# JasperSnoek/spearmint

Hardware: NVIDIA H100
Metric: EI candidates/sec (higher is better)
Workload: dtype f32

## Files before the change

### spearmint_b200/csrc/predict_tc.cu

```cuda
#include <cuda_fp16.h>
#include <cuda.h>

#include <algorithm>
#include <vector>
#include <cstdlib>
#include <cstring>

#include "common.cuh"
#include "tc_common.cuh"

namespace smk {

__global__ void __launch_bounds__(256, 2) trtri_finalize_kernel(int Npad, int ldx, int K, const float* __restrict__ winv,
                                                                 float* X) {
  using C = Cfg<float>;
  constexpr int NB = C::NB, TM = C::TM, TN = C::TN;
  extern __shared__ __align__(16) unsigned char smem_raw[];
  TileSmem<float>& sm = *reinterpret_cast<TileSmem<float>*>(smem_raw);
  float (*Ts)[NB + kPad] = reinterpret_cast<float (*)[NB + kPad]>(smem_raw + sizeof(TileSmem<float>));
  const int nblk = Npad / NB, J = blockIdx.x, s = blockIdx.y;
  const int tid = threadIdx.x, ty = tid >> 4, tx = tid & 15;
  const float* W = winv + ((long)s * nblk + K) * NB * NB;
  float* Xt = X + (long)s * ldx * ldx + (long)K * NB * ldx + (long)J * NB;
  float acc[TM][TN];
// ... 77 lines not shown
  long e = (long)blockIdx.x * blockDim.x + threadIdx.x;
  if (e >= total) return;
  long per = (long)ld * ld;
  int r = (int)((e % per) / ld), c = (int)(e % ld);
  float x = (c <= r && r < Npad) ? X[e] : 0.f;
  float h = tf32_hi(x);
  hi[e] = h;
  lo[e] = x - h;
}

__global__ void __launch_bounds__(256) linv_mv_kernel(int N, int Np, const float* __restrict__ hi,
                                                      const float* __restrict__ lo, const float* __restrict__ y,
                                                      const float* __restrict__ mean, float* __restrict__ t) {
  const int s = blockIdx.y, warp = threadIdx.x >> 5, lane = threadIdx.x & 31;
  const int row = blockIdx.x * 8 + warp;
  if (row >= Np) return;
  const long base = ((long)s * Np + row) * Np;
  const float mu = mean[s];
  float acc = 0.f;
  for (int k = lane; k <= row && k < N; k += 32) acc = fmaf(hi[base + k] + lo[base + k], y[k] - mu, acc);
#pragma unroll
  for (int o = 16; o > 0; o >>= 1) acc += __shfl_xor_sync(0xffffffffu, acc, o);
  if (lane == 0) t[(long)s * Np + row] = (row < N) ? acc : 0.f;
}
__global__ void __launch_bounds__(256) linv_mtv_kernel(int N, int Np, int ld_alpha, const float* __restrict__ hi,
                                                       const float* __restrict__ lo, const float* __restrict__ t,
                                                       float* __restrict__ alpha) {
  __shared__ float red[4][64];
  const int s = blockIdx.y, cl = threadIdx.x & 63, ph = threadIdx.x >> 6;
  const int c = blockIdx.x * 64 + cl;
  const float* th = t + (long)s * Np;
  const long base = (long)s * Np * Np + c;
  float acc = 0.f;
  if (c < N)
    for (int r = (c & ~3) + ph; r < N; r += 4)
      if (r >= c) acc = fmaf(hi[base + (long)r * Np] + lo[base + (long)r * Np], th[r], acc);
  red[ph][cl] = acc;
  __syncthreads();
  if (ph == 0 && c < ld_alpha) alpha[(long)s * ld_alpha + c] = (c < N) ? red[0][cl] + red[1][cl] + red[2][cl] + red[3][cl] : 0.f;
}

__global__ void __launch_bounds__(256) linv_absmax_kernel(long per4, const float4* __restrict__ hi,
                                                          const float4* __restrict__ lo, unsigned* __restrict__ maxbits) {
  const int s = blockIdx.y;
  const float4* h = hi + (long)s * per4;
  const float4* l = lo + (long)s * per4;
  float m = 0.f;
  for (long e = (long)blockIdx.x * blockDim.x + threadIdx.x; e < per4; e += (long)gridDim.x * blockDim.x) {
    float4 a = h[e], b = l[e];
    m = fmaxf(m, fmaxf(fmaxf(fabsf(a.x + b.x), fabsf(a.y + b.y)), fmaxf(fabsf(a.z + b.z), fabsf(a.w + b.w))));
  }
#pragma unroll
  for (int o = 16; o > 0; o >>= 1) m = fmaxf(m, __shfl_xor_sync(0xffffffffu, m, o));
  if ((threadIdx.x & 31) == 0) atomicMax(&maxbits[s], __float_as_uint(m));
}

__global__ void __launch_bounds__(256) linv_pack_f16_kernel(long per4, const float4* __restrict__ hi,
                                                            const float4* __restrict__ lo,
                                                            const unsigned* __restrict__ maxbits, uint2* __restrict__ oh,
                                                            uint2* __restrict__ ol, int* __restrict__ exps) {
  const int s = blockIdx.y;
  const int eb = scale_exp(__uint_as_float(maxbits[s]));
  const float sc = ldexpf(1.f, eb);
  if (blockIdx.x == 0 && threadIdx.x == 0) exps[s] = eb;
  const long base = (long)s * per4;
  for (long e = (long)blockIdx.x * blockDim.x + threadIdx.x; e < per4; e += (long)gridDim.x * blockDim.x) {
    float4 a = hi[base + e], b = lo[base + e];
    __half hh[4], ll[4];
    split16((a.x + b.x) * sc, hh[0], ll[0]);
    split16((a.y + b.y) * sc, hh[1], ll[1]);
    split16((a.z + b.z) * sc, hh[2], ll[2]);
    split16((a.w + b.w) * sc, hh[3], ll[3]);
    oh[base + e] = pack4(hh);
    ol[base + e] = pack4(ll);
  }
}

__global__ void __launch_bounds__(256) alpha_absmax_kernel(int N, int F, int Npad_alpha, const float* __restrict__ alpha,
                                                           int* __restrict__ fexp) {
  __shared__ float red[8];
  const int s = blockIdx.x;
  float m = 0.f;
  for (long e = threadIdx.x; e < (long)F * N; e += blockDim.x) {
    int f = (int)(e / N), n = (int)(e % N);
    m = fmaxf(m, fabsf(alpha[((long)s * F + f) * Npad_alpha + n]));
  }
#pragma unroll
  for (int o = 16; o > 0; o >>= 1) m = fmaxf(m, __shfl_xor_sync(0xffffffffu, m, o));
  if ((threadIdx.x & 31) == 0) red[threadIdx.x >> 5] = m;
  __syncthreads();
  if (threadIdx.x == 0) {
    for (int w = 1; w < 8; ++w) m = fmaxf(m, red[w]);
    fexp[s] = scale_exp(m);
  }
}
__global__ void alpha_pack_f16_kernel(int N, int Np, int F, int Fp, int Npad_alpha, long total,
                                      const float* __restrict__ alpha, const int* __restrict__ fexp,
                                      __half* __restrict__ hi, __half* __restrict__ lo) {
  long e = (long)blockIdx.x * blockDim.x + threadIdx.x;
  if (e >= total) return;
  int n = (int)(e % Np);
  long sf = e / Np;
  int f = (int)(sf % Fp), s = (int)(sf / Fp);
  float x = (f < F && n < N) ? alpha[((long)s * F + f) * Npad_alpha + n] * ldexpf(1.f, fexp[s]) : 0.f;
  split16(x, hi[e], lo[e]);
}

// ... 86 lines not shown
          hh[q] = __floats2half2_rn(v.x, v.y);
          const float2 hf = __half22float2(hh[q]);
          ll[q] = __floats2half2_rn(v.x - hf.x, v.y - hf.y);
        }
        uint2 ph, pl;
        ph.x = *reinterpret_cast<unsigned*>(&hh[0]); ph.y = *reinterpret_cast<unsigned*>(&hh[1]);
        pl.x = *reinterpret_cast<unsigned*>(&ll[0]); pl.y = *reinterpret_cast<unsigned*>(&ll[1]);
        *reinterpret_cast<uint2*>(khi + ok + g * 64 + tx * 4) = ph;
        *reinterpret_cast<uint2*>(klo + ok + g * 64 + tx * 4) = pl;
      }
    }
  }
  if (!al) return;
  __syncthreads();
#pragma unroll
  for (int r = 0; r < 8; ++r) red[tx][tile_row(ty, r)] = mdot[r].x + mdot[r].y;
  __syncthreads();
  if (tid < T) {
    float v = 0.f;
    for (int q = 0; q < 16; ++q) v += red[q][tid];
    int gc = c_begin + c0 + tid;
    if (gc < M) mu[(long)s * ldm + gc] = fmaf(a2, v, mean[s]);
  }
}

namespace tc {
constexpr int BM = 128;
constexpr int BN = 256;
constexpr int BK = 16;
constexpr int BK16 = 32;
constexpr int STAGES = 4;
constexpr int ROW_BYTES = BK * 4;
static_assert(ROW_BYTES == 64 && BK16 * 2 == ROW_BYTES, "operand rows must be one 64B swizzle span in both element types");
constexpr int UK_BYTES = 32;
constexpr int A_BYTES = BM * ROW_BYTES;
constexpr int B_BYTES = BN * ROW_BYTES;
constexpr int STAGE_BYTES = 2 * A_BYTES + 2 * B_BYTES;
constexpr int CONSUMERS = 2;
constexpr int THREADS = (CONSUMERS + 1) * 128;
constexpr int PRODUCER_REGS = 40, CONSUMER_REGS = 232;
static_assert(128 * PRODUCER_REGS + CONSUMERS * 128 * CONSUMER_REGS <= 65536, "register file");
constexpr int SMEM_BYTES = STAGES * STAGE_BYTES + 1024  + 256 ;

struct Args {
  int S, Np, Mc, ntiles, npairs, ngroups, ldp;
  float* partial;
  const float* z;
  float* mpartial;
  float* dbg;
  int F, M, c_begin, ldm;
  const float* mean;
  float* mu_f;
  int f16;
  int a_evict_first;
  const float* amp2;
  const int* bexp;
  int mode;
  int Npad, jb, ncols;
  float* Cmat;
  int K;
  float *xhi, *xlo, *xthi, *xtlo;
};

struct Item { int valid, own, rowA, rowB, k0, nk, s, tile, g, pr; };

template <int CLUSTER>
__device__ __forceinline__ long num_items(const Args& p) {
  return p.mode <= 1 ? (long)p.S * ((p.ntiles + CLUSTER - 1) / CLUSTER) * p.npairs : (long)p.S * p.ntiles;
}
template <int CLUSTER>
__device__ __forceinline__ Item get_item(const Args& p, long w, int h, int rank) {
  Item it;
  it.valid = 0; it.own = 1; it.rowA = it.rowB = it.k0 = it.nk = it.s = it.tile = it.g = it.pr = 0;
  const int bk = p.f16 ? BK16 : BK;
  if (p.mode <= 1) {
    const int ntg = (p.ntiles + CLUSTER - 1) / CLUSTER;
    it.pr = (int)(w % p.npairs);
    const long st = w / p.npairs;
    it.tile = (int)(st % ntg) * CLUSTER + rank;
    it.s = (int)(st / ntg);
    if (it.tile >= p.ntiles) { it.tile = p.ntiles - 1; it.own = 0; }
    it.g = (h == 0) ? it.pr : p.ngroups - 1 - it.pr;
    if (h == 1 && (p.mode == 1 || it.g == it.pr)) return it;
    it.nk = (p.mode == 1) ? p.Np / bk : (it.g + 1) * (BN / bk);
    it.rowA = it.s * p.Mc + it.tile * BM;
    it.rowB = (it.s * p.ngroups + it.g) * BN;
    it.valid = 1;
  } else if (p.mode == 2) {
    if (h == 1) return it;
    it.tile = (int)(w % p.ntiles);
    it.s = (int)(w / p.ntiles);
    it.rowA = it.s * p.Npad + (p.jb + it.tile) * BM;
    it.rowB = it.s * p.Npad + p.jb * BM;
    it.nk = p.jb * BM / bk;
    it.valid = 1;
  } else {
    if (h == 1) return it;
    it.tile = (int)(w % p.ntiles);
    it.s = (int)(w / p.ntiles);
    it.rowA = it.s * BM;
    it.rowB = it.s * p.Np + it.tile * BN;
    it.k0 = it.tile * BN;
    it.nk = (p.K * BM - it.tile * BN) / bk;
    it.valid = 1;
  }
  return it;
}

template <int CLUSTER>
__global__ void __launch_bounds__(THREADS, 1)
predict_tc_kernel(const __grid_constant__ CUtensorMap mAhi, const __grid_constant__ CUtensorMap mAlo,
                  const __grid_constant__ CUtensorMap mBhi, const __grid_constant__ CUtensorMap mBlo, Args p) {
  static_assert(CLUSTER == 1 || CLUSTER == 2, "one CTA, or a pair sharing the B operand");
  extern __shared__ unsigned char smem_raw[];
  unsigned char* base = smem_raw + ((1024u - (smem_u32(smem_raw) & 1023u)) & 1023u);
  uint64_t* bars = reinterpret_cast<uint64_t*>(base + STAGES * STAGE_BYTES);
  uint64_t* full = bars;
  uint64_t* empty = bars + STAGES;

  const int warp = threadIdx.x >> 5, lane = threadIdx.x & 31;
  const int rank = CLUSTER > 1 ? (int)cluster_ctarank() : 0;
  if (threadIdx.x == 0) {
    for (int i = 0; i < STAGES; ++i) { mbar_init(&full[i], 1); mbar_init(&empty[i], CLUSTER * CONSUMERS * 4); }
    asm volatile("fence.mbarrier_init.release.cluster;" ::: "memory");
  }
  if (CLUSTER > 1) cluster_sync();
  else __syncthreads();

  const long nitems = num_items<CLUSTER>(p);
  const long w0 = blockIdx.x / CLUSTER, dw = gridDim.x / CLUSTER;
  const int bk = p.f16 ? BK16 : BK;
  if (warp < 4) {
    asm volatile("setmaxnreg.dec.sync.aligned.u32 %0;" ::"n"(PRODUCER_REGS));
    if (warp == 0 && lane == 0) {
      const uint64_t hintA = (p.mode == 0 && !p.a_evict_first) ? 0x1000000000000000ull : 0x12F0000000000000ull;
      const uint64_t hintB = 0x14F0000000000000ull;
      int stage = 0;
      uint32_t phase = 0;
      for (long w = w0; w < nitems; w += dw) {
        for (int h = 0; h < 2; ++h) {
          const Item it = get_item<CLUSTER>(p, w, h, rank);
          if (!it.valid) break;
          for (int kc = 0; kc < it.nk; ++kc) {
            mbar_wait_relaxed(&empty[stage], phase ^ 1, 64);
            unsigned char* sb = base + stage * STAGE_BYTES;
            const int kk = it.k0 + kc * bk;
            mbar_expect_tx(&full[stage], STAGE_BYTES);
            tma_load_2d(&mAhi, &full[stage], sb, kk, it.rowA, hintA);
            tma_load_2d(&mAlo, &full[stage], sb + A_BYTES, kk, it.rowA, hintA);
            if (CLUSTER == 1) {
              tma_load_2d(&mBhi, &full[stage], sb + 2 * A_BYTES, kk, it.rowB, hintB);
              tma_load_2d(&mBlo, &full[stage], sb + 2 * A_BYTES + B_BYTES, kk, it.rowB, hintB);
            } else {
              const int hb = rank * (BN / CLUSTER);
              const uint16_t all = (1u << CLUSTER) - 1;
              tma_load_2d_multicast(&mBhi, &full[stage], sb + 2 * A_BYTES + hb * ROW_BYTES, kk, it.rowB + hb, all, hintB);
              tma_load_2d_multicast(&mBlo, &full[stage], sb + 2 * A_BYTES + B_BYTES + hb * ROW_BYTES, kk, it.rowB + hb,
                                    all, hintB);
            }
            if (++stage == STAGES) { stage = 0; phase ^= 1; }
          }
        }
      }
    }
    if (CLUSTER > 1) cluster_sync();
    return;
  }

  asm volatile("setmaxnreg.inc.sync.aligned.u32 %0;" ::"n"(CONSUMER_REGS));
  const int wg = (warp >> 2) - 1;
  const int r0 = wg * 64 + (warp & 3) * 16 + (lane >> 2);
  const int cq = 2 * (lane & 3);
  const uint32_t a_off = (uint32_t)wg * 64 * ROW_BYTES;
  auto release = [&](int st) {
    if (CLUSTER == 1) mbar_arrive(&empty[st]);
    else
#pragma unroll
      for (int r = 0; r < CLUSTER; ++r) mbar_arrive_cluster(&empty[st], r);
  };
  float d[BN / 2];
  int stage = 0;
  uint32_t phase = 0;
  for (long w = w0; w < nitems; w += dw) {
    float acc[2] = {0.f, 0.f}, accm[2] = {0.f, 0.f};
    const Item it0 = get_item<CLUSTER>(p, w, 0, rank);
    for (int h = 0; h < 2; ++h) {
      const Item it = get_item<CLUSTER>(p, w, h, rank);
      if (!it.valid) break;
      int prev = -1;
      for (int kc = 0; kc < it.nk; ++kc) {
        mbar_wait(&full[stage], phase);
        const uint32_t sa = smem_u32(base + stage * STAGE_BYTES);
        const uint64_t ahi = wgmma_desc_sw64(sa + a_off), alo = wgmma_desc_sw64(sa + A_BYTES + a_off);
        const uint64_t bhi = wgmma_desc_sw64(sa + 2 * A_BYTES), blo = wgmma_desc_sw64(sa + 2 * A_BYTES + B_BYTES);
        wgmma_fence();
        if (p.f16) {
#pragma unroll
          for (int k = 0; k < ROW_BYTES / UK_BYTES; ++k) {
            const uint64_t ko = (uint64_t)((k * UK_BYTES) >> 4);
            wgmma_f16_n256(d, alo + ko, bhi + ko, (kc | k) ? 1u : 0u);
            wgmma_f16_n256(d, ahi + ko, blo + ko, 1u);
            wgmma_f16_n256(d, ahi + ko, bhi + ko, 1u);
          }
        } else {
#pragma unroll
          for (int k = 0; k < ROW_BYTES / UK_BYTES; ++k) {
            const uint64_t ko = (uint64_t)((k * UK_BYTES) >> 4);
            wgmma_tf32_n256(d, alo + ko, bhi + ko, (kc | k) ? 1u : 0u);
            wgmma_tf32_n256(d, ahi + ko, blo + ko, 1u);
            wgmma_tf32_n256(d, ahi + ko, bhi + ko, 1u);
          }
        }
        wgmma_commit();
        wgmma_wait<1>();
        if (prev >= 0 && lane == 0) release(prev);
        prev = stage;
        if (++stage == STAGES) { stage = 0; phase ^= 1; }
      }
      wgmma_wait<0>();
      wgmma_hold(d);
      if (prev >= 0 && lane == 0) release(prev);
      if (!it.own) continue;
      const float scl = p.f16 ? ldexpf(1.f, -(kx_exp(p.amp2[it.s]) + p.bexp[it.s])) : 1.f;
      if (p.mode == 0) {
        const float* zrow = p.z ? p.z + (long)it.s * p.Np + it.g * BN : nullptr;
#pragma unroll
        for (int nb = 0; nb < BN / 8; ++nb) {
          const int c = nb * 8 + cq;
          const float2 z2 = zrow ? __ldg(reinterpret_cast<const float2*>(zrow + c)) : make_float2(0.f, 0.f);
#pragma unroll
          for (int rh = 0; rh < 2; ++rh) {
            const float v0 = d[nb * 4 + rh * 2] * scl, v1 = d[nb * 4 + rh * 2 + 1] * scl;
            acc[rh] = fmaf(v0, v0, acc[rh]);
            acc[rh] = fmaf(v1, v1, acc[rh]);
            accm[rh] = fmaf(v0, z2.x, accm[rh]);
            accm[rh] = fmaf(v1, z2.y, accm[rh]);
            if (p.dbg) {
              float* o = p.dbg + ((long)it.s * p.Mc + it.tile * BM + r0 + 8 * rh) * p.Np + it.g * BN + c;
              o[0] = v0;
              o[1] = v1;
            }
          }
        }
      } else if (p.mode == 1) {
        const float mu0 = p.mean[it.s];
#pragma unroll
        for (int rh = 0; rh < 2; ++rh) {
          const int gc = p.c_begin + it.tile * BM + r0 + 8 * rh;
          if (gc >= p.M) continue;
#pragma unroll
          for (int nb = 0; nb < BN / 8; ++nb)
#pragma unroll
            for (int e = 0; e < 2; ++e) {
              const int f = it.g * BN + nb * 8 + cq + e;
              if (f < p.F) p.mu_f[((long)it.s * p.F + f) * p.ldm + gc] = fmaf(d[nb * 4 + rh * 2 + e], scl, mu0);
            }
        }
      } else if (p.mode == 2) {
#pragma unroll
        for (int nb = 0; nb < BN / 8; ++nb) {
          const int c = nb * 8 + cq;
          if (c >= p.ncols) continue;
#pragma unroll
          for (int rh = 0; rh < 2; ++rh) {
            float2* cp = reinterpret_cast<float2*>(
// ... 238 lines not shown
  for (int r = 0; r < TM; ++r)
#pragma unroll
    for (int c = 0; c < TN; ++c) acc[r][c] = 0.f;
  TileGemm<float, Lay::KContig, Lay::MContig, false>::run(acc, W, NB, Lk, Npad, NB, sm);
  const long off = (long)s * NB * Npad + (long)J * NB;
#pragma unroll
  for (int r = 0; r < TM; ++r)
#pragma unroll
    for (int g = 0; g < TN / 4; ++g) {
      V4<float> h, l;
#pragma unroll
      for (int e = 0; e < 4; ++e) {
        float x = acc[r][g * 4 + e];
        h.v[e] = tf32_hi(x);
        l.v[e] = tf32_lo(x, h.v[e]);
      }
      const long o = off + (long)tile_row(ty, r) * Npad + g * 64 + tx * 4;
      st4(lthi + o, h);
      st4(ltlo + o, l);
    }
}

__global__ void trtri_diag_store_kernel(int Npad, int Np, int K, const float* __restrict__ winv, float* __restrict__ xhi,
                                        float* __restrict__ xlo, float* __restrict__ xthi, float* __restrict__ xtlo) {
  constexpr int NB = 128;
  const int s = blockIdx.y, nblk = Npad / NB;
  const float* W = winv + ((long)s * nblk + K) * NB * NB;
  for (int e = blockIdx.x * blockDim.x + threadIdx.x; e < NB * NB; e += gridDim.x * blockDim.x) {
    int i = e / NB, k = e % NB;
    float x = W[e], h = tf32_hi(x), l = x - h;
    long o = ((long)s * Np + (long)K * NB + i) * Np + (long)K * NB + k;
    long ot = ((long)s * Np + (long)K * NB + k) * Np + (long)K * NB + i;
    xhi[o] = h; xlo[o] = l; xthi[ot] = h; xtlo[ot] = tf32_lo(x, h);
  }
}

size_t trtri_tc_workspace_bytes(int Npad, int Np, int S) {
  return (2 * (size_t)S * Np * Np + 2 * (size_t)S * 128 * Npad) * sizeof(float);
}

int potrf_lower_batched_tc(int, int, float*, float*, int*, float*, float*, cudaStream_t, cudaEvent_t*);
void potrf_winv_block(int, int, int, const float*, float*, cudaStream_t);

static int trtri_tc_run(int Npad, int Np, int S, const float* L, float* winv, float* linv_hi, float* linv_lo,
                        void* workspace, size_t workspace_bytes, cudaStream_t st, cudaEvent_t* blk_done) {
  if (Npad <= 0 || Npad % kNpadMult) return -1;
  if (Np < Npad || Np % tc::BN) return -2;
  if (S <= 0) return -3;
  if (!L || !winv || !linv_hi || !linv_lo) return -4;
  if (!workspace || workspace_bytes < trtri_tc_workspace_bytes(Npad, Np, S)) return -8;
  float* xthi = reinterpret_cast<float*>(workspace);
  float* xtlo = xthi + (size_t)S * Np * Np;
  float* lthi = xtlo + (size_t)S * Np * Np;
  float* ltlo = lthi + (size_t)S * 128 * Npad;
  const size_t xb = (size_t)S * Np * Np * sizeof(float);
  cudaMemsetAsync(linv_hi, 0, xb, st);
  cudaMemsetAsync(linv_lo, 0, xb, st);
  cudaMemsetAsync(xthi, 0, 2 * xb, st);
  CUtensorMap mAhi, mAlo, mBhi, mBlo;
  if (tc::make_map(&mAhi, lthi, (uint64_t)S * 128, Npad, tc::BM) || tc::make_map(&mAlo, ltlo, (uint64_t)S * 128, Npad, tc::BM) ||
      tc::make_map(&mBhi, xthi, (uint64_t)S * Np, Np, tc::BN) || tc::make_map(&mBlo, xtlo, (uint64_t)S * Np, Np, tc::BN))
    return 1999;
  static bool attr = false;
  if (!attr) {
    cudaFuncSetAttribute(tc::predict_tc_kernel<1>, cudaFuncAttributeMaxDynamicSharedMemorySize, tc::SMEM_BYTES);
    attr = true;
  }
  const int nblk = Npad / 128;
  timing_begin("trtri_kernel", st);
  for (int K = 0; K < nblk; ++K) {
    if (blk_done) {
      cudaStreamWaitEvent(st, blk_done[K], 0);
      potrf_winv_block(Npad, S, K, L, winv, st);
    }
    trtri_diag_store_kernel<<<dim3(8, S), 256, 0, st>>>(Npad, Np, K, winv, linv_hi, linv_lo, xthi, xtlo);
    count_launch();
    if (K == 0) continue;
    trtri_lt_kernel<<<dim3(K, S), 256, 0, st>>>(Npad, K, L, winv, lthi, ltlo);
    tc::Args a;
    tc_args_init(a);
    a.mode = 3; a.S = S; a.Np = Np; a.Npad = Npad; a.K = K;
    a.ntiles = (K * 128 + tc::BN - 1) / tc::BN; a.npairs = 1; a.ngroups = 1;
    a.xhi = linv_hi; a.xlo = linv_lo; a.xthi = xthi; a.xtlo = xtlo;
    long nitems = (long)S * a.ntiles;
    int grid = (int)std::min<long>(nitems, num_sms());
    tc::predict_tc_kernel<1><<<grid, tc::THREADS, tc::SMEM_BYTES, st>>>(mAhi, mAlo, mBhi, mBlo, a);
    count_launch(2);
  }
  timing_end(st);
  return check_launch("trtri_split_tc");
}
// ... 7 lines not shown
                   float* linv_lo, void* tws, size_t tws_bytes, cudaStream_t st) {
  if (Npad <= 0 || Npad % kNpadMult) return -1;
  static cudaStream_t aux = nullptr;
  static cudaEvent_t ev_in = nullptr, ev_out = nullptr;
  static std::vector<cudaEvent_t> blk;
  if (!aux) {
    cudaStreamCreateWithFlags(&aux, cudaStreamNonBlocking);
    cudaEventCreateWithFlags(&ev_in, cudaEventDisableTiming);
    cudaEventCreateWithFlags(&ev_out, cudaEventDisableTiming);
  }
  const int nblk = Npad / 128;
  while ((int)blk.size() < nblk) {
    cudaEvent_t e;
    cudaEventCreateWithFlags(&e, cudaEventDisableTiming);
    blk.push_back(e);
  }
  cudaEventRecord(ev_in, st);
  cudaStreamWaitEvent(aux, ev_in, 0);
  int rc = potrf_lower_batched_tc(Npad, S, A, winv, info, lhi, llo, st, blk.data());
  if (rc) return rc;
  rc = trtri_tc_run(Npad, Np, S, A, winv, linv_hi, linv_lo, tws, tws_bytes, aux, blk.data());
  cudaEventRecord(ev_out, aux);
  cudaStreamWaitEvent(st, ev_out, 0);
  return rc;
}

int linv_pack_f16(int Np, int S, const float* linv_hi, const float* linv_lo, __half* out_hi, __half* out_lo, int* exps,
                  cudaStream_t st) {
  if (Np <= 0 || Np % tc::BN) return -1;
  if (S <= 0) return -2;
  if (!linv_hi || !linv_lo || !out_hi || !out_lo || !exps) return -3;
  unsigned* maxbits = reinterpret_cast<unsigned*>(exps + S);
  cudaMemsetAsync(maxbits, 0, sizeof(unsigned) * S, st);
  const long per4 = (long)Np * Np / 4;
  const int gx = (int)std::min<long>((per4 + 255) / 256, 4L * num_sms());
  timing_begin("linv_pack_f16", st);
  linv_absmax_kernel<<<dim3(gx, S), 256, 0, st>>>(per4, reinterpret_cast<const float4*>(linv_hi),
                                                  reinterpret_cast<const float4*>(linv_lo), maxbits);
  linv_pack_f16_kernel<<<dim3(gx, S), 256, 0, st>>>(per4, reinterpret_cast<const float4*>(linv_hi),
                                                    reinterpret_cast<const float4*>(linv_lo), maxbits,
                                                    reinterpret_cast<uint2*>(out_hi), reinterpret_cast<uint2*>(out_lo), exps);
  timing_end(st);
  count_launch(2);
  return check_launch("linv_pack_f16");
}

int linv_alpha(int N, int Np, int S, const float* linv_hi, const float* linv_lo, const float* y, const float* mean,
               float* alpha, int ld_alpha, float* tmp, cudaStream_t st) {
  if (N <= 0 || Np < N) return -1;
  if (S <= 0) return -3;
  if (!linv_hi || !linv_lo || !y || !mean || !alpha || !tmp) return -4;
  if (ld_alpha < N) return -9;
  linv_mv_kernel<<<dim3((Np + 7) / 8, S), 256, 0, st>>>(N, Np, linv_hi, linv_lo, y, mean, tmp);
  linv_mtv_kernel<<<dim3((ld_alpha + 63) / 64, S), 256, 0, st>>>(N, Np, ld_alpha, linv_hi, linv_lo, tmp, alpha);
  count_launch(2);
  return check_launch("linv_alpha");
}

static bool tc_overlap_enabled() {
  static int v = -1;
  if (v < 0) { const char* e = getenv("SMK_TC_OVERLAP"); v = (e && e[0] == '1') ? 1 : 0; }
  return v == 1;
}
static size_t tc_chunk_cands(int Np, int M, int S, size_t budget) {
  size_t per_cand = (size_t)S * Np * 2 * sizeof(__half);
  size_t mpad = ((size_t)M + 127) / 128 * 128;
  size_t mc = budget / per_cand;
  if (mc >= mpad) return mpad;
  if (tc_overlap_enabled()) mc = (budget / 2) / per_cand;
  mc = mc / 128 * 128;
  if (mc < 128) mc = 128;
  return mc;
// ... 140 lines not shown
  void* kws = reinterpret_cast<void*>(fexp + S);
  float* mu_partial = gen_tc ? kxt_tc_mu_partial(kws, Np, Mc, S, M, D) : nullptr;
  const float* gen_alpha = z ? nullptr : alpha;
  const bool pre = pregenerated && z && nbuf == 1 && g_pregen.valid && g_pregen.ws == workspace && g_pregen.M == M &&
                   g_pregen.S == S && g_pregen.Np == Np && g_pregen.N == N;
  if (pregenerated && !pre) return -21;
  if (g_pregen.valid && g_pregen.ws == workspace) {
    cudaStreamWaitEvent(st, g_pregen.done, 0);
    g_pregen.valid = false;
  }
  if (!pre && gen_tc) {
    int rc = kxt_tc_prepare(kws, N, Np, M, Mc, D, S, X, Cc, st);
    if (rc) return rc;
  }
  CUtensorMap mFhi, mFlo;
  if (fant) {
    const long total = (long)S * Fp * Np;
    alpha_absmax_kernel<<<S, 256, 0, st>>>(N, F, Npad_alpha, alpha_f, fexp);
    alpha_pack_f16_kernel<<<(unsigned)((total + 255) / 256), 256, 0, st>>>(N, Np, F, Fp, Npad_alpha, total, alpha_f, fexp,
                                                                           ahi, alo);
    count_launch(2);
    if (tc::make_map_h(&mFhi, ahi, (uint64_t)S * Fp, Np, tc::BN / tc::kPredictCluster) ||
        tc::make_map_h(&mFlo, alo, (uint64_t)S * Fp, Np, tc::BN / tc::kPredictCluster))
      return 1999;
  }

  CUtensorMap mAhi[2], mAlo[2], mBhi, mBlo;
  for (int b = 0; b < nbuf; ++b) {
    __half* kh = kbase + (size_t)b * 2 * kelems;
    if (tc::make_map_h(&mAhi[b], kh, (uint64_t)S * Mc, Np, tc::BM) ||
        tc::make_map_h(&mAlo[b], kh + kelems, (uint64_t)S * Mc, Np, tc::BM))
      return 1999;
  }
  if (tc::make_map_h(&mBhi, linv_hi, (uint64_t)S * Np, Np, tc::BN / tc::kPredictCluster) ||
      tc::make_map_h(&mBlo, linv_lo, (uint64_t)S * Np, Np, tc::BN / tc::kPredictCluster))
    return 1999;
  static cudaStream_t aux = nullptr;
  static cudaEvent_t ev_fork = nullptr, ev_kxt[2] = {nullptr, nullptr}, ev_mma[2] = {nullptr, nullptr};
  if (!aux) {
    cudaStreamCreateWithFlags(&aux, cudaStreamNonBlocking);
    cudaEventCreateWithFlags(&ev_fork, cudaEventDisableTiming);
    for (int i = 0; i < 2; ++i) {
      cudaEventCreateWithFlags(&ev_kxt[i], cudaEventDisableTiming);
      cudaEventCreateWithFlags(&ev_mma[i], cudaEventDisableTiming);
    }
  }
  const bool overlap = (nbuf == 2);
  cudaStream_t kst = overlap ? aux : st;
  if (overlap) {
    cudaEventRecord(ev_fork, st);
    cudaStreamWaitEvent(aux, ev_fork, 0);
  }
  int ci = 0;
  for (int c_begin = 0; c_begin < M; c_begin += Mc, ++ci) {
    const int b = overlap ? (ci & 1) : 0;
    __half* kh = kbase + (size_t)b * 2 * kelems;
    const int mc_used = min(Mc, ((M - c_begin) + 127) / 128 * 128);
    if (overlap && ci >= 2) cudaStreamWaitEvent(aux, ev_mma[b], 0);
    if (!(pre && ci == 0)) {
      timing_begin("kxt_kernel", kst);
      if (gen_tc) {
        int rc = kxt_tc(kws, kind, N, Np, M, c_begin, Mc, mc_used, D, S, inv_ls, amp2, gen_alpha, Npad_alpha, kh, kh + kelems, kst);
        if (rc) return rc;
      } else {
        kxt_kernel<<<dim3(mc_used / 128, S), 256, 0, kst>>>(kind, N, Np, M, c_begin, Mc, D, X, Cc, inv_ls, amp2, mean,
                                                            gen_alpha, Npad_alpha, kh, kh + kelems, mu, ldm);
      }
      timing_end(kst);
// ... 36 lines not shown
```

### spearmint_b200/csrc/tc_common.cuh

```cuda
#pragma once
#include <cuda_fp16.h>
#include <cuda.h>

#include <cstdint>

namespace smk {

__host__ __device__ __forceinline__ int scale_exp(float amax) {
  int e;
  frexpf(amax * 1.00001f, &e);
  return 15 - e;
}
__device__ __forceinline__ int kx_exp(float amp2) { return scale_exp(amp2 * 1.000001f); }
__device__ __forceinline__ void split16(float x, __half& h, __half& l) {
  h = __float2half_rn(x);
  l = __float2half_rn(x - __half2float(h));
}
__device__ __forceinline__ uint2 pack4(const __half (&v)[4]) {
  __half2 a = __halves2half2(v[0], v[1]), b = __halves2half2(v[2], v[3]);
  uint2 r;
  r.x = *reinterpret_cast<unsigned*>(&a);
  r.y = *reinterpret_cast<unsigned*>(&b);
  return r;
}
// ... 149 lines not shown
      : "l"(a), "l"(b), "r"(scale_d));
}
__device__ __forceinline__ void wgmma_tf32_n256(float (&d)[128], uint64_t a, uint64_t b, uint32_t scale_d) {
  asm volatile(
      "{\n\t.reg .pred p;\n\t"
      "setp.ne.b32 p, %130, 0;\n\t"
      "wgmma.mma_async.sync.aligned.m64n256k8.f32.tf32.tf32 "
      "{%0, %1, %2, %3, %4, %5, %6, %7, %8, %9, %10, %11, %12, %13, %14, %15, "
      "%16, %17, %18, %19, %20, %21, %22, %23, %24, %25, %26, %27, %28, %29, %30, %31, "
      "%32, %33, %34, %35, %36, %37, %38, %39, %40, %41, %42, %43, %44, %45, %46, %47, "
      "%48, %49, %50, %51, %52, %53, %54, %55, %56, %57, %58, %59, %60, %61, %62, %63, "
      "%64, %65, %66, %67, %68, %69, %70, %71, %72, %73, %74, %75, %76, %77, %78, %79, "
      "%80, %81, %82, %83, %84, %85, %86, %87, %88, %89, %90, %91, %92, %93, %94, %95, "
      "%96, %97, %98, %99, %100, %101, %102, %103, %104, %105, %106, %107, %108, %109, %110, %111, "
      "%112, %113, %114, %115, %116, %117, %118, %119, %120, %121, %122, %123, %124, %125, %126, %127}, "
      "%128, %129, p, 1, 1;\n\t}"
      : "+f"(d[0]), "+f"(d[1]), "+f"(d[2]), "+f"(d[3]), "+f"(d[4]), "+f"(d[5]), "+f"(d[6]), "+f"(d[7]), "+f"(d[8]), "+f"(d[9]), "+f"(d[10]), "+f"(d[11]), "+f"(d[12]), "+f"(d[13]), "+f"(d[14]), "+f"(d[15]), "+f"(d[16]), "+f"(d[17]), "+f"(d[18]), "+f"(d[19]), "+f"(d[20]), "+f"(d[21]), "+f"(d[22]), "+f"(d[23]), "+f"(d[24]), "+f"(d[25]), "+f"(d[26]), "+f"(d[27]), "+f"(d[28]), "+f"(d[29]), "+f"(d[30]), "+f"(d[31]), "+f"(d[32]), "+f"(d[33]), "+f"(d[34]), "+f"(d[35]), "+f"(d[36]), "+f"(d[37]), "+f"(d[38]), "+f"(d[39]), "+f"(d[40]), "+f"(d[41]), "+f"(d[42]), "+f"(d[43]), "+f"(d[44]), "+f"(d[45]), "+f"(d[46]), "+f"(d[47]), "+f"(d[48]), "+f"(d[49]), "+f"(d[50]), "+f"(d[51]), "+f"(d[52]), "+f"(d[53]), "+f"(d[54]), "+f"(d[55]), "+f"(d[56]), "+f"(d[57]), "+f"(d[58]), "+f"(d[59]), "+f"(d[60]), "+f"(d[61]), "+f"(d[62]), "+f"(d[63]), "+f"(d[64]), "+f"(d[65]), "+f"(d[66]), "+f"(d[67]), "+f"(d[68]), "+f"(d[69]), "+f"(d[70]), "+f"(d[71]), "+f"(d[72]), "+f"(d[73]), "+f"(d[74]), "+f"(d[75]), "+f"(d[76]), "+f"(d[77]), "+f"(d[78]), "+f"(d[79]), "+f"(d[80]), "+f"(d[81]), "+f"(d[82]), "+f"(d[83]), "+f"(d[84]), "+f"(d[85]), "+f"(d[86]), "+f"(d[87]), "+f"(d[88]), "+f"(d[89]), "+f"(d[90]), "+f"(d[91]), "+f"(d[92]), "+f"(d[93]), "+f"(d[94]), "+f"(d[95]), "+f"(d[96]), "+f"(d[97]), "+f"(d[98]), "+f"(d[99]), "+f"(d[100]), "+f"(d[101]), "+f"(d[102]), "+f"(d[103]), "+f"(d[104]), "+f"(d[105]), "+f"(d[106]), "+f"(d[107]), "+f"(d[108]), "+f"(d[109]), "+f"(d[110]), "+f"(d[111]), "+f"(d[112]), "+f"(d[113]), "+f"(d[114]), "+f"(d[115]), "+f"(d[116]), "+f"(d[117]), "+f"(d[118]), "+f"(d[119]), "+f"(d[120]), "+f"(d[121]), "+f"(d[122]), "+f"(d[123]), "+f"(d[124]), "+f"(d[125]), "+f"(d[126]), "+f"(d[127])
      : "l"(a), "l"(b), "r"(scale_d));
}
__device__ __forceinline__ void wgmma_f16_n128(float (&d)[64], uint64_t a, uint64_t b, uint32_t scale_d) {
  asm volatile(
      "{\n\t.reg .pred p;\n\t"
      "setp.ne.b32 p, %66, 0;\n\t"
      "wgmma.mma_async.sync.aligned.m64n128k16.f32.f16.f16 "
      "{%0, %1, %2, %3, %4, %5, %6, %7, %8, %9, %10, %11, %12, %13, %14, %15, "
      "%16, %17, %18, %19, %20, %21, %22, %23, %24, %25, %26, %27, %28, %29, %30, %31, "
      "%32, %33, %34, %35, %36, %37, %38, %39, %40, %41, %42, %43, %44, %45, %46, %47, "
      "%48, %49, %50, %51, %52, %53, %54, %55, %56, %57, %58, %59, %60, %61, %62, %63}, "
      "%64, %65, p, 1, 1, 0, 0;\n\t}"
      : "+f"(d[0]), "+f"(d[1]), "+f"(d[2]), "+f"(d[3]), "+f"(d[4]), "+f"(d[5]), "+f"(d[6]), "+f"(d[7]), "+f"(d[8]), "+f"(d[9]), "+f"(d[10]), "+f"(d[11]), "+f"(d[12]), "+f"(d[13]), "+f"(d[14]), "+f"(d[15]), "+f"(d[16]), "+f"(d[17]), "+f"(d[18]), "+f"(d[19]), "+f"(d[20]), "+f"(d[21]), "+f"(d[22]), "+f"(d[23]), "+f"(d[24]), "+f"(d[25]), "+f"(d[26]), "+f"(d[27]), "+f"(d[28]), "+f"(d[29]), "+f"(d[30]), "+f"(d[31]), "+f"(d[32]), "+f"(d[33]), "+f"(d[34]), "+f"(d[35]), "+f"(d[36]), "+f"(d[37]), "+f"(d[38]), "+f"(d[39]), "+f"(d[40]), "+f"(d[41]), "+f"(d[42]), "+f"(d[43]), "+f"(d[44]), "+f"(d[45]), "+f"(d[46]), "+f"(d[47]), "+f"(d[48]), "+f"(d[49]), "+f"(d[50]), "+f"(d[51]), "+f"(d[52]), "+f"(d[53]), "+f"(d[54]), "+f"(d[55]), "+f"(d[56]), "+f"(d[57]), "+f"(d[58]), "+f"(d[59]), "+f"(d[60]), "+f"(d[61]), "+f"(d[62]), "+f"(d[63])
      : "l"(a), "l"(b), "r"(scale_d));
}

}
}
```

### spearmint_b200/engine.py

```python
import ctypes as C
import os

import numpy as np
import scipy.stats as sps
import torch

from . import _lib
from ._lib import KINDS, check, fn, ptr

JITTER = 1e-6
CONSTRAINT_NOISE = 1e-3


def _ceil(x, m):
    return ((x + m - 1) // m) * m


class HyperBatch(object):

    def __init__(self, hyper_samples, kind, device, dtype):
        S = len(hyper_samples)
        D = len(np.atleast_1d(hyper_samples[0][3]))
        mean = np.array([h[0] for h in hyper_samples], dtype=np.float64)
        noise = np.array([h[1] for h in hyper_samples], dtype=np.float64)
# ... 4 lines not shown
        host = np.concatenate([mean, noise, amp2, (1.0 / ls).ravel()])
        dev = torch.from_numpy(host).to(device=device, dtype=dtype, non_blocking=False)
        self.S, self.D = S, D
        self.mean, self.noise, self.amp2 = dev[:S], dev[S:2 * S], dev[2 * S:3 * S]
        self.inv_ls = dev[3 * S:].view(S, D)
        self.host_mean, self.host_noise, self.host_amp2, self.host_ls = mean, noise, amp2, ls
        self.nbytes = host.size * (8 if dtype == torch.float64 else 4)

    def slice(self, a, b):
        o = object.__new__(HyperBatch)
        o.S, o.D = b - a, self.D
        o.mean, o.noise, o.amp2, o.inv_ls = self.mean[a:b], self.noise[a:b], self.amp2[a:b], self.inv_ls[a:b]
        o.host_mean, o.host_noise = self.host_mean[a:b], self.host_noise[a:b]
        o.host_amp2, o.host_ls = self.host_amp2[a:b], self.host_ls[a:b]
        o.nbytes = 0
        return o


class Factor(object):

    def __init__(self, eng, kind, X, hb, L=None, winv=None, info=None, factor_impl=None):
        self.eng, self.kind, self.hb = eng, kind, hb
        self.factor_impl = factor_impl or eng.factor_impl
        self.X = X
        self.N, self.D = X.shape
        self.Npad = _ceil(self.N, 128)
        S, dt, dev = hb.S, eng.dtype, eng.device
        NB = eng.NB
        self._owned = []
        self.L = L if L is not None else self._take((S, self.Npad, self.Npad))
        self.winv = winv if winv is not None else self._take((S, self.Npad // NB, NB, NB))
        self.info = info if info is not None else torch.zeros((S,), dtype=torch.int32, device=dev)
        st = eng.stream()
        check(fn("smk_cov_build", dt)(KINDS[kind], self.N, self.N, self.D, S, ptr(X), None, ptr(hb.inv_ls),
                                      ptr(hb.amp2), ptr(hb.noise), ptr(self.L), self.Npad, st), "cov_build")
        if self.factor_impl == "tc" and dt == torch.float32 and self.Npad >= 256:
            L = _lib.lib()
            nb = 2 * S * self.Npad * self.Npad * 4
            ws = eng.take((nb,), torch.uint8)
            if eng.fused_inverse:
                Np = L.smk_tc_np(self.N)
                hi = self._take((S, Np, Np), torch.float32)
                lo = self._take((S, Np, Np), torch.float32)
                nt = L.smk_trtri_tc_workspace_bytes(self.Npad, Np, S)
                wt = eng.take((nt,), torch.uint8)
                check(L.smk_potrf_trtri_tc_f32(self.Npad, Np, S, ptr(self.L), ptr(self.winv), ptr(self.info), ptr(ws), nb,
                                               ptr(hi), ptr(lo), ptr(wt), nt, st), "potrf_trtri_tc")
                eng.give(ws, wt)
                self._linv = (hi, lo, Np)
            else:
                eng.give(ws)
                check(L.smk_potrf_lower_batched_tc_f32(self.Npad, S, ptr(self.L), ptr(self.winv), ptr(self.info),
                                                       ptr(ws), nb, st), "potrf_tc")
        else:
            check(fn("smk_potrf_lower_batched", dt)(self.Npad, S, ptr(self.L), ptr(self.winv), ptr(self.info), st),
                  "potrf")

    def _take(self, shape, dtype=None):
        t = self.eng.take(shape, dtype)
        self._owned.append(t)
        return t

    def __del__(self):
        try:
            self.eng.give(*self._owned)
        except Exception:
            pass

    def linv(self):
# ... 1003 lines not shown
```

Baseline: 215,100.

## Exploit triangular Linv diagonal block: shrink wgmma N and skip zero B loads

Over the last 8 k-stages (the diagonal block of the triangular inverse factor), the B tile is loaded in 32-row pieces in reversed order. Each stage then issues wgmma with progressively narrower N (256 down to 32), skipping columns known to be zero. In the final half, the rank-0 CTA of the 2-CTA cluster skips its multicast B loads, and the transaction byte count is reduced to match. The epilogue remaps accumulator columns to the reversed layout. This adds an 8-way switch over template-specialised MMA widths and makes the TMA box smaller, which risks more TMA instructions and bugs with the fp16-only path when mode 0 runs with tf32.

```diff
diff --git a/spearmint_b200/csrc/predict_tc.cu b/spearmint_b200/csrc/predict_tc.cu
--- a/spearmint_b200/csrc/predict_tc.cu
+++ b/spearmint_b200/csrc/predict_tc.cu
@@ -326,6 +326,11 @@
 constexpr int STAGES = 4;
 constexpr int ROW_BYTES = BK * 4;
 static_assert(ROW_BYTES == 64 && BK16 * 2 == ROW_BYTES, "operand rows must be one 64B swizzle span in both element types");
+constexpr int kLinvRowBlock = 32;
+static_assert(BN == 256 && BN / BK16 == 8 && kLinvRowBlock == BK16, "a diagonal block is 8 stages of 32 rows of k");
+__host__ __device__ constexpr int linv_acc_col(int row) {
+  return BN - kLinvRowBlock * (row / kLinvRowBlock + 1) + row % kLinvRowBlock;
+}
 constexpr int UK_BYTES = 32;
 constexpr int A_BYTES = BM * ROW_BYTES;
 constexpr int B_BYTES = BN * ROW_BYTES;
@@ -439,15 +444,26 @@
             mbar_wait_relaxed(&empty[stage], phase ^ 1, 64);
             unsigned char* sb = base + stage * STAGE_BYTES;
             const int kk = it.k0 + kc * bk;
-            mbar_expect_tx(&full[stage], STAGE_BYTES);
+            const bool zero_half = CLUSTER == 2 && p.mode == 0 && kc >= it.nk - BN / BK16 / 2;
+            mbar_expect_tx(&full[stage], zero_half ? STAGE_BYTES - B_BYTES : STAGE_BYTES);
             tma_load_2d(&mAhi, &full[stage], sb, kk, it.rowA, hintA);
             tma_load_2d(&mAlo, &full[stage], sb + A_BYTES, kk, it.rowA, hintA);
+            const int hb = rank * (BN / CLUSTER);
+            const uint16_t all = (1u << CLUSTER) - 1;
             if (CLUSTER == 1) {
               tma_load_2d(&mBhi, &full[stage], sb + 2 * A_BYTES, kk, it.rowB, hintB);
               tma_load_2d(&mBlo, &full[stage], sb + 2 * A_BYTES + B_BYTES, kk, it.rowB, hintB);
+            } else if (p.mode == 0) {
+              if (!(zero_half && rank == 0)) {
+                unsigned char* sbB = sb + 2 * A_BYTES + linv_acc_col(hb) * ROW_BYTES;
+#pragma unroll
+                for (int j = 0; j < BN / CLUSTER / kLinvRowBlock; ++j) {
+                  const int r = hb + j * kLinvRowBlock, sr = -j * kLinvRowBlock * ROW_BYTES;
+                  tma_load_2d_multicast(&mBhi, &full[stage], sbB + sr, kk, it.rowB + r, all, hintB);
+                  tma_load_2d_multicast(&mBlo, &full[stage], sbB + B_BYTES + sr, kk, it.rowB + r, all, hintB);
+                }
+              }
             } else {
-              const int hb = rank * (BN / CLUSTER);
-              const uint16_t all = (1u << CLUSTER) - 1;
               tma_load_2d_multicast(&mBhi, &full[stage], sb + 2 * A_BYTES + hb * ROW_BYTES, kk, it.rowB + hb, all, hintB);
               tma_load_2d_multicast(&mBlo, &full[stage], sb + 2 * A_BYTES + B_BYTES + hb * ROW_BYTES, kk, it.rowB + hb,
                                     all, hintB);
@@ -488,7 +504,10 @@
         const uint64_t ahi = wgmma_desc_sw64(sa + a_off), alo = wgmma_desc_sw64(sa + A_BYTES + a_off);
         const uint64_t bhi = wgmma_desc_sw64(sa + 2 * A_BYTES), blo = wgmma_desc_sw64(sa + 2 * A_BYTES + B_BYTES);
         wgmma_fence();
-        if (p.f16) {
+        const int qd = p.mode == 0 ? kc - (it.nk - BN / BK16) : -1;
+        if (qd >= 0) {
+          mma3_f16_stage_cols(qd, d, ahi, alo, bhi, blo, kc ? 1u : 0u);
+        } else if (p.f16) {
 #pragma unroll
           for (int k = 0; k < ROW_BYTES / UK_BYTES; ++k) {
             const uint64_t ko = (uint64_t)((k * UK_BYTES) >> 4);
@@ -520,11 +539,11 @@
         const float* zrow = p.z ? p.z + (long)it.s * p.Np + it.g * BN : nullptr;
 #pragma unroll
         for (int nb = 0; nb < BN / 8; ++nb) {
-          const int c = nb * 8 + cq;
+          const int c = nb * 8 + cq, ab = linv_acc_col(nb * 8) / 8;
           const float2 z2 = zrow ? __ldg(reinterpret_cast<const float2*>(zrow + c)) : make_float2(0.f, 0.f);
 #pragma unroll
           for (int rh = 0; rh < 2; ++rh) {
-            const float v0 = d[nb * 4 + rh * 2] * scl, v1 = d[nb * 4 + rh * 2 + 1] * scl;
+            const float v0 = d[ab * 4 + rh * 2] * scl, v1 = d[ab * 4 + rh * 2 + 1] * scl;
             acc[rh] = fmaf(v0, v0, acc[rh]);
             acc[rh] = fmaf(v1, v1, acc[rh]);
             accm[rh] = fmaf(v0, z2.x, accm[rh]);
@@ -1139,8 +1158,8 @@
         tc::make_map_h(&mAlo[b], kh + kelems, (uint64_t)S * Mc, Np, tc::BM))
       return 1999;
   }
-  if (tc::make_map_h(&mBhi, linv_hi, (uint64_t)S * Np, Np, tc::BN / tc::kPredictCluster) ||
-      tc::make_map_h(&mBlo, linv_lo, (uint64_t)S * Np, Np, tc::BN / tc::kPredictCluster))
+  if (tc::make_map_h(&mBhi, linv_hi, (uint64_t)S * Np, Np, tc::kLinvRowBlock) ||
+      tc::make_map_h(&mBlo, linv_lo, (uint64_t)S * Np, Np, tc::kLinvRowBlock))
     return 1999;
   static cudaStream_t aux = nullptr;
   static cudaEvent_t ev_fork = nullptr, ev_kxt[2] = {nullptr, nullptr}, ev_mma[2] = {nullptr, nullptr};
diff --git a/spearmint_b200/csrc/tc_common.cuh b/spearmint_b200/csrc/tc_common.cuh
--- a/spearmint_b200/csrc/tc_common.cuh
+++ b/spearmint_b200/csrc/tc_common.cuh
@@ -205,5 +205,70 @@
       : "l"(a), "l"(b), "r"(scale_d));
 }
 
-}
-}
+template <int N>
+__device__ __forceinline__ void wgmma_f16_n(float (&d)[128], uint64_t a, uint64_t b, uint32_t scale_d);
+#define SMK_ACC_8(o) "+f"(d[o]), "+f"(d[o + 1]), "+f"(d[o + 2]), "+f"(d[o + 3]), "+f"(d[o + 4]), "+f"(d[o + 5]), \
+                     "+f"(d[o + 6]), "+f"(d[o + 7])
+#define SMK_ACC_16(o) SMK_ACC_8(o), SMK_ACC_8(o + 8)
+#define SMK_ACC_R16 SMK_ACC_16(0)
+#define SMK_ACC_R32 SMK_ACC_R16, SMK_ACC_16(16)
+#define SMK_ACC_R48 SMK_ACC_R32, SMK_ACC_16(32)
+#define SMK_ACC_R64 SMK_ACC_R48, SMK_ACC_16(48)
+#define SMK_ACC_R80 SMK_ACC_R64, SMK_ACC_16(64)
+#define SMK_ACC_R96 SMK_ACC_R80, SMK_ACC_16(80)
+#define SMK_ACC_R112 SMK_ACC_R96, SMK_ACC_16(96)
+#define SMK_REG_R16 "%0, %1, %2, %3, %4, %5, %6, %7, %8, %9, %10, %11, %12, %13, %14, %15"
+#define SMK_REG_R32 SMK_REG_R16 ", %16, %17, %18, %19, %20, %21, %22, %23, %24, %25, %26, %27, %28, %29, %30, %31"
+#define SMK_REG_R48 SMK_REG_R32 ", %32, %33, %34, %35, %36, %37, %38, %39, %40, %41, %42, %43, %44, %45, %46, %47"
+#define SMK_REG_R64 SMK_REG_R48 ", %48, %49, %50, %51, %52, %53, %54, %55, %56, %57, %58, %59, %60, %61, %62, %63"
+#define SMK_REG_R80 SMK_REG_R64 ", %64, %65, %66, %67, %68, %69, %70, %71, %72, %73, %74, %75, %76, %77, %78, %79"
+#define SMK_REG_R96 SMK_REG_R80 ", %80, %81, %82, %83, %84, %85, %86, %87, %88, %89, %90, %91, %92, %93, %94, %95"
+#define SMK_REG_R112 SMK_REG_R96 ", %96, %97, %98, %99, %100, %101, %102, %103, %104, %105, %106, %107, %108, %109, %110, %111"
+#define SMK_WGMMA_F16_N(N, R, RA, RB, RS)                                                                          \
+  template <>                                                                                                      \
+  __device__ __forceinline__ void wgmma_f16_n<N>(float (&d)[128], uint64_t a, uint64_t b, uint32_t scale_d) {    \
+    asm volatile("{\n\t.reg .pred p;\n\tsetp.ne.b32 p, %" #RS ", 0;\n\t"                                           \
+                 "wgmma.mma_async.sync.aligned.m64n" #N "k16.f32.f16.f16 {" SMK_REG_R##R "}, %" #RA ", %" #RB      \
+                 ", p, 1, 1, 0, 0;\n\t}"                                                                           \
+                 : SMK_ACC_R##R                                                                                    \
+                 : "l"(a), "l"(b), "r"(scale_d));                                                                  \
+  }
+SMK_WGMMA_F16_N(224, 112, 112, 113, 114)
+SMK_WGMMA_F16_N(192, 96, 96, 97, 98)
+SMK_WGMMA_F16_N(160, 80, 80, 81, 82)
+SMK_WGMMA_F16_N(128, 64, 64, 65, 66)
+SMK_WGMMA_F16_N(96, 48, 48, 49, 50)
+SMK_WGMMA_F16_N(64, 32, 32, 33, 34)
+SMK_WGMMA_F16_N(32, 16, 16, 17, 18)
+template <>
+__device__ __forceinline__ void wgmma_f16_n<256>(float (&d)[128], uint64_t a, uint64_t b, uint32_t scale_d) {
+  wgmma_f16_n256(d, a, b, scale_d);
+}
+
+template <int Q>
+__device__ __forceinline__ void mma3_f16_stage_cols(float (&d)[128], uint64_t ahi, uint64_t alo, uint64_t bhi,
+                                                    uint64_t blo, uint32_t scale_d) {
+  constexpr int N = 256 - 32 * Q;
+#pragma unroll
+  for (int k = 0; k < 2; ++k) {
+    wgmma_f16_n<N>(d, alo + 2 * k, bhi + 2 * k, k ? 1u : scale_d);
+    wgmma_f16_n<N>(d, ahi + 2 * k, blo + 2 * k, 1u);
+    wgmma_f16_n<N>(d, ahi + 2 * k, bhi + 2 * k, 1u);
+  }
+}
+__device__ __forceinline__ void mma3_f16_stage_cols(int q, float (&d)[128], uint64_t ahi, uint64_t alo, uint64_t bhi,
+                                                    uint64_t blo, uint32_t scale_d) {
+  switch (q) {
+    case 0: mma3_f16_stage_cols<0>(d, ahi, alo, bhi, blo, scale_d); break;
+    case 1: mma3_f16_stage_cols<1>(d, ahi, alo, bhi, blo, scale_d); break;
+    case 2: mma3_f16_stage_cols<2>(d, ahi, alo, bhi, blo, scale_d); break;
+    case 3: mma3_f16_stage_cols<3>(d, ahi, alo, bhi, blo, scale_d); break;
+    case 4: mma3_f16_stage_cols<4>(d, ahi, alo, bhi, blo, scale_d); break;
+    case 5: mma3_f16_stage_cols<5>(d, ahi, alo, bhi, blo, scale_d); break;
+    case 6: mma3_f16_stage_cols<6>(d, ahi, alo, bhi, blo, scale_d); break;
+    default: mma3_f16_stage_cols<7>(d, ahi, alo, bhi, blo, scale_d); break;
+  }
+}
+
+}
+}
```

Measured after the change: 215,500, median of 6. No clear change (+0.2%).

## Exploit lower-triangular structure in Linv pack, zeroing, and covariance build

Applied to the files above, without the earlier changes.

The full-matrix memsets of the inverse buffers are replaced by a kernel that zeros only the upper block region. The absmax and f16 pack kernels now read only the lower block-triangular columns of each row and write zeros elsewhere. The covariance build switches to a lower-only variant on the TC path. The mtv loop drops its per-iteration branch and is unrolled, and the mode-3 tile scheduler is remapped to a serpentine, sample-interleaved order. Correctness now depends on the remaining code never reading the skipped upper regions, and on the new smk_cov_build_lower symbol existing in the library.

```diff
diff --git a/spearmint_b200/csrc/predict_tc.cu b/spearmint_b200/csrc/predict_tc.cu
--- a/spearmint_b200/csrc/predict_tc.cu
+++ b/spearmint_b200/csrc/predict_tc.cu
@@ -133,47 +133,62 @@
   const float* th = t + (long)s * Np;
   const long base = (long)s * Np * Np + c;
   float acc = 0.f;
-  if (c < N)
-    for (int r = (c & ~3) + ph; r < N; r += 4)
-      if (r >= c) acc = fmaf(hi[base + (long)r * Np] + lo[base + (long)r * Np], th[r], acc);
+  if (c < N) {
+    int r = (c & ~3) + ph;
+    if (r < c) r += 4;
+#pragma unroll 8
+    for (; r < N; r += 4) acc = fmaf(hi[base + (long)r * Np] + lo[base + (long)r * Np], th[r], acc);
+  }
   red[ph][cl] = acc;
   __syncthreads();
   if (ph == 0 && c < ld_alpha) alpha[(long)s * ld_alpha + c] = (c < N) ? red[0][cl] + red[1][cl] + red[2][cl] + red[3][cl] : 0.f;
 }
 
-__global__ void __launch_bounds__(256) linv_absmax_kernel(long per4, const float4* __restrict__ hi,
+__device__ __forceinline__ int linv_lower_cols4(int r, int Np) { return min(Np, (r / 128 + 1) * 128) / 4; }
+
+__global__ void __launch_bounds__(256) linv_absmax_kernel(int Np, const float4* __restrict__ hi,
                                                           const float4* __restrict__ lo, unsigned* __restrict__ maxbits) {
-  const int s = blockIdx.y;
-  const float4* h = hi + (long)s * per4;
-  const float4* l = lo + (long)s * per4;
+  const int s = blockIdx.y, n4 = Np / 4;
   float m = 0.f;
-  for (long e = (long)blockIdx.x * blockDim.x + threadIdx.x; e < per4; e += (long)gridDim.x * blockDim.x) {
-    float4 a = h[e], b = l[e];
-    m = fmaxf(m, fmaxf(fmaxf(fabsf(a.x + b.x), fabsf(a.y + b.y)), fmaxf(fabsf(a.z + b.z), fabsf(a.w + b.w))));
+  for (int r = blockIdx.x; r < Np; r += gridDim.x) {
+    const long row = ((long)s * Np + r) * n4;
+    const int c4 = linv_lower_cols4(r, Np);
+    for (int c = threadIdx.x; c < c4; c += blockDim.x) {
+      const float4 a = hi[row + c], b = lo[row + c];
+      m = fmaxf(m, fmaxf(fmaxf(fabsf(a.x + b.x), fabsf(a.y + b.y)), fmaxf(fabsf(a.z + b.z), fabsf(a.w + b.w))));
+    }
   }
 #pragma unroll
   for (int o = 16; o > 0; o >>= 1) m = fmaxf(m, __shfl_xor_sync(0xffffffffu, m, o));
   if ((threadIdx.x & 31) == 0) atomicMax(&maxbits[s], __float_as_uint(m));
 }
 
-__global__ void __launch_bounds__(256) linv_pack_f16_kernel(long per4, const float4* __restrict__ hi,
+__global__ void __launch_bounds__(256) linv_pack_f16_kernel(int Np, const float4* __restrict__ hi,
                                                             const float4* __restrict__ lo,
                                                             const unsigned* __restrict__ maxbits, uint2* __restrict__ oh,
                                                             uint2* __restrict__ ol, int* __restrict__ exps) {
-  const int s = blockIdx.y;
+  const int s = blockIdx.y, n4 = Np / 4;
   const int eb = scale_exp(__uint_as_float(maxbits[s]));
   const float sc = ldexpf(1.f, eb);
   if (blockIdx.x == 0 && threadIdx.x == 0) exps[s] = eb;
-  const long base = (long)s * per4;
-  for (long e = (long)blockIdx.x * blockDim.x + threadIdx.x; e < per4; e += (long)gridDim.x * blockDim.x) {
-    float4 a = hi[base + e], b = lo[base + e];
-    __half hh[4], ll[4];
-    split16((a.x + b.x) * sc, hh[0], ll[0]);
-    split16((a.y + b.y) * sc, hh[1], ll[1]);
-    split16((a.z + b.z) * sc, hh[2], ll[2]);
-    split16((a.w + b.w) * sc, hh[3], ll[3]);
-    oh[base + e] = pack4(hh);
-    ol[base + e] = pack4(ll);
+  for (int r = blockIdx.x; r < Np; r += gridDim.x) {
+    const long row = ((long)s * Np + r) * n4;
+    const int c4 = linv_lower_cols4(r, Np);
+    for (int c = threadIdx.x; c < n4; c += blockDim.x) {
+      uint2 ph = make_uint2(0u, 0u), pl = make_uint2(0u, 0u);
+      if (c < c4) {
+        const float4 a = hi[row + c], b = lo[row + c];
+        __half hh[4], ll[4];
+        split16((a.x + b.x) * sc, hh[0], ll[0]);
+        split16((a.y + b.y) * sc, hh[1], ll[1]);
+        split16((a.z + b.z) * sc, hh[2], ll[2]);
+        split16((a.w + b.w) * sc, hh[3], ll[3]);
+        ph = pack4(hh);
+        pl = pack4(ll);
+      }
+      oh[row + c] = ph;
+      ol[row + c] = pl;
+    }
   }
 }
 
@@ -390,8 +405,10 @@
     it.valid = 1;
   } else {
     if (h == 1) return it;
-    it.tile = (int)(w % p.ntiles);
-    it.s = (int)(w / p.ntiles);
+    const long G = gridDim.x, rnd = w / G, b = w % G;
+    const long v = ((rnd & 1) && (rnd + 1) * G <= (long)p.S * p.ntiles) ? rnd * G + G - 1 - b : w;
+    it.tile = (int)(v / p.S);
+    it.s = (int)(v % p.S);
     it.rowA = it.s * BM;
     it.rowB = it.s * p.Np + it.tile * BN;
     it.k0 = it.tile * BN;
@@ -829,7 +846,18 @@
     long o = ((long)s * Np + (long)K * NB + i) * Np + (long)K * NB + k;
     long ot = ((long)s * Np + (long)K * NB + k) * Np + (long)K * NB + i;
     xhi[o] = h; xlo[o] = l; xthi[ot] = h; xtlo[ot] = tf32_lo(x, h);
-  }
+    if (K & 1) { xthi[o - NB] = 0.f; xtlo[o - NB] = 0.f; }
+  }
+}
+
+__global__ void __launch_bounds__(256) linv_zero_upper_kernel(int Npad, int Np, float* __restrict__ xhi,
+                                                              float* __restrict__ xlo) {
+  const int r = blockIdx.x, s = blockIdx.y;
+  const int c0 = r < Npad ? (r / 128 + 1) * 128 : 0;
+  float4* h = reinterpret_cast<float4*>(xhi + ((long)s * Np + r) * Np);
+  float4* l = reinterpret_cast<float4*>(xlo + ((long)s * Np + r) * Np);
+  const float4 z = make_float4(0.f, 0.f, 0.f, 0.f);
+  for (int c = c0 / 4 + threadIdx.x; c < Np / 4; c += blockDim.x) { h[c] = z; l[c] = z; }
 }
 
 size_t trtri_tc_workspace_bytes(int Npad, int Np, int S) {
@@ -850,10 +878,8 @@
   float* xtlo = xthi + (size_t)S * Np * Np;
   float* lthi = xtlo + (size_t)S * Np * Np;
   float* ltlo = lthi + (size_t)S * 128 * Npad;
-  const size_t xb = (size_t)S * Np * Np * sizeof(float);
-  cudaMemsetAsync(linv_hi, 0, xb, st);
-  cudaMemsetAsync(linv_lo, 0, xb, st);
-  cudaMemsetAsync(xthi, 0, 2 * xb, st);
+  linv_zero_upper_kernel<<<dim3(Np, S), 256, 0, st>>>(Npad, Np, linv_hi, linv_lo);
+  count_launch();
   CUtensorMap mAhi, mAlo, mBhi, mBlo;
   if (tc::make_map(&mAhi, lthi, (uint64_t)S * 128, Npad, tc::BM) || tc::make_map(&mAlo, ltlo, (uint64_t)S * 128, Npad, tc::BM) ||
       tc::make_map(&mBhi, xthi, (uint64_t)S * Np, Np, tc::BN) || tc::make_map(&mBlo, xtlo, (uint64_t)S * Np, Np, tc::BN))
@@ -927,12 +953,11 @@
   if (!linv_hi || !linv_lo || !out_hi || !out_lo || !exps) return -3;
   unsigned* maxbits = reinterpret_cast<unsigned*>(exps + S);
   cudaMemsetAsync(maxbits, 0, sizeof(unsigned) * S, st);
-  const long per4 = (long)Np * Np / 4;
-  const int gx = (int)std::min<long>((per4 + 255) / 256, 4L * num_sms());
+  const int gx = std::min(Np, 4 * num_sms());
   timing_begin("linv_pack_f16", st);
-  linv_absmax_kernel<<<dim3(gx, S), 256, 0, st>>>(per4, reinterpret_cast<const float4*>(linv_hi),
+  linv_absmax_kernel<<<dim3(gx, S), 256, 0, st>>>(Np, reinterpret_cast<const float4*>(linv_hi),
                                                   reinterpret_cast<const float4*>(linv_lo), maxbits);
-  linv_pack_f16_kernel<<<dim3(gx, S), 256, 0, st>>>(per4, reinterpret_cast<const float4*>(linv_hi),
+  linv_pack_f16_kernel<<<dim3(gx, S), 256, 0, st>>>(Np, reinterpret_cast<const float4*>(linv_hi),
                                                     reinterpret_cast<const float4*>(linv_lo), maxbits,
                                                     reinterpret_cast<uint2*>(out_hi), reinterpret_cast<uint2*>(out_lo), exps);
   timing_end(st);
diff --git a/spearmint_b200/engine.py b/spearmint_b200/engine.py
--- a/spearmint_b200/engine.py
+++ b/spearmint_b200/engine.py
@@ -60,9 +60,14 @@
         self.winv = winv if winv is not None else self._take((S, self.Npad // NB, NB, NB))
         self.info = info if info is not None else torch.zeros((S,), dtype=torch.int32, device=dev)
         st = eng.stream()
-        check(fn("smk_cov_build", dt)(KINDS[kind], self.N, self.N, self.D, S, ptr(X), None, ptr(hb.inv_ls),
-                                      ptr(hb.amp2), ptr(hb.noise), ptr(self.L), self.Npad, st), "cov_build")
-        if self.factor_impl == "tc" and dt == torch.float32 and self.Npad >= 256:
+        tc = self.factor_impl == "tc" and dt == torch.float32 and self.Npad >= 256
+        if tc:
+            check(fn("smk_cov_build_lower", dt)(KINDS[kind], self.N, self.D, S, ptr(X), ptr(hb.inv_ls), ptr(hb.amp2),
+                                                ptr(hb.noise), ptr(self.L), self.Npad, st), "cov_build")
+        else:
+            check(fn("smk_cov_build", dt)(KINDS[kind], self.N, self.N, self.D, S, ptr(X), None, ptr(hb.inv_ls),
+                                          ptr(hb.amp2), ptr(hb.noise), ptr(self.L), self.Npad, st), "cov_build")
+        if tc:
             L = _lib.lib()
             nb = 2 * S * self.Npad * self.Npad * 4
             ws = eng.take((nb,), torch.uint8)
```

New measurement: 214,100 before, 220,200 after, median of 6. +2.9%, better.
